# bifurcationkit/BifurcationKit.jl

Measured on NVIDIA H100. Metric: continuation steps/sec (SH2d PALC), higher is better.
Workload: dtype f64

## Files before the change

### bifurcationkit.jl_b200/csrc/bk_common.cuh

```cuda
#pragma once
#include <cuda_runtime.h>
#include <stdint.h>
#include <stdlib.h>
#include <string>
#include <unordered_map>
#include <vector>
#include "../../include/bk200.h"
#include <nvtx3/nvToolsExt.h>

struct BkRange {
  explicit BkRange(const char* name) { nvtxRangePushA(name); }
  ~BkRange() { nvtxRangePop(); }
};

#define BK_MAX_PAR 8
#define BK_NSM_FALLBACK 132

struct OpDesc {
  int kind;
  int nx, ny, nz;
  double cx, cy, cz;
  double par[BK_MAX_PAR];
  const double* u;
  double a0, a1;
// ... 34 lines not shown
  const double* sp;
  double a0, a1, l, nu;
  double spc;
};
#define PW_D 1

struct Precond {
  int kind = BK_PC_NONE;
  double a0 = 0, a1 = 0;
  double* lam[3] = {nullptr, nullptr, nullptr};
  int ttype[3] = {0, 0, 0};
  int fast[3] = {0, 0, 0};
  double2* ftw[3] = {nullptr, nullptr, nullptr};
  double2* fom[3] = {nullptr, nullptr, nullptr};
  double2* flam2[3] = {nullptr, nullptr, nullptr};
  bkg::Plan gplan[3] = {};
  double2* gwl[3] = {nullptr, nullptr, nullptr};
  double2* gph[3] = {nullptr, nullptr, nullptr};
  double* work = nullptr;
  double* work2 = nullptr;
  double* tri = nullptr;
  double2* tdft = nullptr;
  double po_r = 0, po_nu = 0, po_T = 0;
};

struct BkKindTraits {
  int ndims;
  int fields;
  int extra;
  bool jac_sym;
// ... 237 lines not shown
```

### bifurcationkit.jl_b200/csrc/bk_ctx.cu

```cuda
#include <cstdio>
#include <cstring>
#include <map>
#include <mutex>
#include <new>
#include "bk_common.cuh"

int bk_fail(bk_ctx* c, int code, const char* what, const char* file, int line) {
  if (c) {
    char buf[512];
    snprintf(buf, sizeof buf, "%s (%s:%d)", what, file, line);
    c->err = buf;
  }
  return code;
}

void bk_grant_smem(int device, const void* kern, size_t bytes) {
  static std::mutex mu;
  static std::map<std::pair<int, const void*>, size_t> granted;
  std::lock_guard<std::mutex> lk(mu);
  size_t& cur = granted[{device, kern}];
  if (bytes <= cur) return;
  cudaFuncSetAttribute(kern, cudaFuncAttributeMaxDynamicSharedMemorySize, (int)bytes);
  if (bytes > 48 * 1024) cudaFuncSetAttribute(kern, cudaFuncAttributePreferredSharedMemoryCarveout, 100);
  cur = bytes;
// ... 140 lines not shown
  }
  if (kind == BK_SH2D_PERIODIC) BK_TRY(bk_periodic_setup(c));
  BK_CUDA(c, cudaStreamSynchronize(c->stream));
  return BK_OK;
}

extern "C" int32_t bk_ctx_destroy(bk_ctx* c) {
  if (!c) return BK_OK;
  cudaSetDevice(c->device);
  if (c->stream) cudaStreamSynchronize(c->stream);
  double* bufs[] = {c->u_state, c->V, c->w, c->z, c->r, c->scales, c->gcoef, c->hcols, c->hcols2, c->partials,
                    c->red_out, c->phi, c->xpi, c->fcache, c->pc.work, c->pc.work2, c->pc.tri, c->Q, c->Q2, c->eig_dev};
  for (double* b : bufs)
    if (b) cudaFree(b);
  for (int d = 0; d < 3; ++d) {
    void* tabs[] = {c->pc.lam[d], c->pc.ftw[d], c->pc.fom[d], c->pc.flam2[d], c->pc.gwl[d], c->pc.gph[d]};
    for (void* t : tabs)
      if (t) cudaFree(t);
  }
  if (c->pc.tdft) cudaFree(c->pc.tdft);
  if (c->counters) cudaFree(c->counters);
  for (auto& kv : c->vec_live) cudaFree(kv.first);
  for (double* b : c->stage)
    if (b) cudaFree(b);
  for (double* b : c->tmp)
    if (b) cudaFree(b);
  if (c->h_pinned) cudaFreeHost(c->h_pinned);
  if (c->red_pinned) cudaFreeHost(c->red_pinned);
  if (c->coef_pinned) cudaFreeHost(c->coef_pinned);
  if (c->host_pinned) cudaFreeHost(c->host_pinned);
  if (c->eig_pinned) cudaFreeHost(c->eig_pinned);
// ... 253 lines not shown
```

### bifurcationkit.jl_b200/csrc/bk_fft_fast.cuh

```cuda
#pragma once
#include "bk_common.cuh"
#include "bk_async.cuh"

namespace bkf {

template <int LOGN_, int LOGE_>
struct Cfg {
  static constexpr int LOGN = LOGN_, LOGE = LOGE_;
  static constexpr int N = 1 << LOGN, E = 1 << LOGE, T = N / E;
  static constexpr int F = LOGN / LOGE, RB = LOGN % LOGE;
  static constexpr int NP = F + (RB ? 1 : 0);
  static constexpr int PP = (T >= 32) ? 2 : 64 / T;
  static constexpr int THREADS = T * PP;
  static constexpr int PB = LOGE == 5 ? (LOGN >= 10 ? 5 : 4) : LOGE == 4 ? 4 : LOGE == 3 ? ((LOGN == 9 || LOGN == 10) ? 3 : 0) : 0;
  __host__ __device__ static constexpr int pad(int i) { return i + (i >> 2) + (PB ? (i >> PB) : 0); }
  static constexpr int TPSM = LOGE == 5 ? 256 : LOGE == 4 ? 512 : LOGE == 3 ? 768 : 1024;
  static constexpr int MINB = TPSM / THREADS > 0 ? TPSM / THREADS : 1;
  static constexpr int MINB_P = MINB > 1 ? MINB - 1 : 1;
  static constexpr int NB = LOGE == 2 ? (LOGN <= 6 ? 0 : LOGN <= 8 ? 4 : LOGN <= 10 ? 6 : 8)
                          : LOGE == 3 ? (LOGN <= 6 ? 0 : LOGN <= 9 ? 3 : 6)
                          : LOGE == 4 ? (LOGN <= 8 ? 0 : 4)
                                      : (LOGN <= 10 ? 0 : 5);
  __host__ __device__ static constexpr int padn(int k) { return k + (k >> 2) + (NB ? (k >> NB) : 0); }
  static constexpr int SLOTS_POS = pad(N - 1) + 1, SLOTS_NAT = padn(N - 1) + 1;
  static constexpr int SLOTS = SLOTS_POS > SLOTS_NAT ? SLOTS_POS : SLOTS_NAT;
  static constexpr size_t SMEM_DATA = sizeof(double2) * (size_t)SLOTS * PP;
  __host__ __device__ static constexpr int logr(int p) { return p < F ? LOGE : RB; }
  __host__ __device__ static constexpr int logNp(int p) { return LOGN - LOGE * p; }
  __host__ __device__ static constexpr int logMp(int p) { return logNp(p) - logr(p); }
  __host__ __device__ static constexpr int tw_off(int p) {
    int o = 0;
    for (int q = 0; q < p; ++q) o += ((1 << logr(q)) - 1) << logMp(q);
    return o;
  }
  static constexpr int TW_TOTAL = tw_off(NP);
  static constexpr size_t SMEM = SMEM_DATA + sizeof(double2) * ((size_t)TW_TOTAL + N);
  static constexpr size_t SMEM_FUSED = SMEM + sizeof(double2) * (size_t)N;
  static_assert(LOGN >= LOGE + 1 && LOGN <= 11, "line length out of range");
  static_assert(THREADS <= 1024, "CTA too large");
};

template <class C>
__host__ __device__ inline int k_of_pos(int p) {
  int k = 0, sh = 0;
  for (int q = 0; q < C::NP; ++q) {
    const int d = (p >> C::logMp(q)) & ((1 << C::logr(q)) - 1);
    k |= d << sh;
    sh += C::logr(q);
  }
  return k;
}
template <class C>
// ... 80 lines not shown
    bfly_inv<H, S0, ESZ>(a);
    bfly_inv<H, S0 + H, ESZ>(a);
#pragma unroll
    for (int i = 0; i < H; ++i) {
      const double2 u = a[S0 + i], t = mul_w32<true>(a[S0 + i + H], i * (32 / R));
      a[S0 + i] = cadd(u, t);
      a[S0 + i + H] = csub(u, t);
    }
  }
}

struct Tables {
  const double2* tw;
  const double2* om;
  const double2* lam2;
};
template <class C, bool FUSED>
__device__ __forceinline__ Tables stage_tables(const Tables& g, double2* sm, unsigned long long* bar) {
  Tables t;
  double2* stw = sm + (size_t)C::SLOTS * C::PP;
  double2* som = stw + C::TW_TOTAL;
  double2* slam = som + C::N;
  if (threadIdx.x == 0) {
    mbar_init(bar, 1);
    fence_mbar_init();
    constexpr unsigned twb = 16u * C::TW_TOTAL, nb = 16u * C::N;
    mbar_arrive_expect_tx(bar, twb + nb + (FUSED ? nb : 0u));
    if (twb) bulk_g2s(stw, g.tw, twb, bar);
    bulk_g2s(som, g.om, nb, bar);
    if (FUSED) bulk_g2s(slam, g.lam2, nb, bar);
  }
  t.tw = stw;
  t.om = som;
  t.lam2 = slam;
  return t;
}

struct Geom {
  long long es;
  long long os;
  int nb;
  int nouter;
};

struct Symbol {
  const double* lam_b;
  const double* lam_o;
  double shift;
  double scale;
// ... 128 lines not shown
    for (int i = 0; i < C::E; ++i) a[i] = make_double2(v0 ? __ldg(base + (long long)row_of<C>(i, tau) * es) : 0.0, 0.0);
  }
}
template <class C>
__device__ __forceinline__ void strided_store(const double2 (&a)[C::E], double* __restrict__ base, long long es, int tau, bool v0,
                                              bool v1) {
  if (v1) {
#pragma unroll
    for (int i = 0; i < C::E; ++i) *reinterpret_cast<double2*>(base + (long long)row_of<C>(i, tau) * es) = a[i];
  } else if (v0) {
#pragma unroll
    for (int i = 0; i < C::E; ++i) base[(long long)row_of<C>(i, tau) * es] = a[i].x;
  }
}

#define BKF_BOUNDS(C, PERIODIC) __launch_bounds__(C::THREADS, (PERIODIC) ? C::MINB_P : C::MINB)

__device__ __forceinline__ double rcp_nr(double x) {
  double r;
  asm("rcp.approx.ftz.f64 %0, %1;" : "=d"(r) : "d"(x));
  double e = fma(-x, r, 1.0);
  r = fma(r, e, r);
  e = fma(-x, r, 1.0);
  return fma(r, e, r);
}
__device__ __forceinline__ double per_symbol(const Symbol& sy, double lam) {
  const double t = 1.0 + lam, l1 = t * t;
  return sy.neg ? -sy.scale * l1 : sy.scale * rcp_nr(l1 + sy.shift);
}

template <class C, int MODE>
static __global__ void BKF_BOUNDS(C, MODE == 3) k_strided(const double* __restrict__ in, double* __restrict__ out, Geom g, Tables tbg, Symbol sy) {
  extern __shared__ __align__(128) double2 sm_fast[];
  __shared__ __align__(8) unsigned long long tbar;
  double2* sm = sm_fast;
  const Tables tb = stage_tables<C, MODE == 2 || MODE == 3>(tbg, sm, &tbar);
  const int tid = threadIdx.x, pr = tid % C::PP, tau = tid / C::PP;
  __syncthreads();
  bk_pdl_sync();
  const int col = (blockIdx.x * C::PP + pr) * 2, o = blockIdx.y;
  const bool v0 = col < g.nb, v1 = col + 1 < g.nb;
  const long long off = (long long)o * g.os + col;
  if ((MODE == 2 || MODE == 3) && sy.tail_n > 0 && blockIdx.x == 0 && blockIdx.y == 0 && tid < sy.tail_n)
    sy.tail_dst[tid] = sy.tail_src[tid];
  double2 a[C::E];
  if (MODE == 3) {
#pragma unroll
    for (int i = 0; i < C::E; ++i) {
      const double* p = in + off + (long long)(i * C::T + tau) * g.es;
      a[i] = v1 ? __ldg(reinterpret_cast<const double2*>(p)) : make_double2(v0 ? __ldg(p) : 0.0, 0.0);
    }
    mbar_wait(&tbar, 0);
    fwd_passes<C, 0>(a, sm, tb, tau, pr);
    const bool nyq = blockIdx.x == 0 && pr == 0;
    if (blockIdx.x == 0) {
      park<C>(a, sm, tau, pr);
      __syncthreads();
      if (nyq) {
        const double l0 = __ldg(sy.lam_b), ln = __ldg(sy.lam_b + (g.nb >> 1));
#pragma unroll
        for (int reg = 0; reg < C::E; ++reg) {
          int k;
          const double2 z = a[reg], zp = partner<C>(sm, reg_pos<C>(tau, reg), pr, k);
          const double ly = tb.lam2[reg * C::T + tau].x;
          const double s0 = per_symbol(sy, l0 + ly), sn = per_symbol(sy, ln + ly);
          const double hp = 0.5 * (s0 + sn), hm = 0.5 * (s0 - sn);
          a[reg] = make_double2(fma(hp, z.x, hm * zp.x), fma(hp, z.y, -(hm * zp.y)));
        }
      }
      __syncthreads();
    }
    if (!nyq) {
      const double lq = v0 ? __ldg(sy.lam_b + (col >> 1)) : 0.0;
#pragma unroll
      for (int reg = 0; reg < C::E; ++reg) {
        const double s = per_symbol(sy, lq + tb.lam2[reg * C::T + tau].x);
        a[reg] = make_double2(s * a[reg].x, s * a[reg].y);
      }
    }
    inv_passes<C, C::NP - 1>(a, sm, tb, tau, pr);
#pragma unroll
    for (int i = 0; i < C::E; ++i) {
      double* p = out + off + (long long)(i * C::T + tau) * g.es;
      if (v1) *reinterpret_cast<double2*>(p) = a[i];
      else if (v0) *p = a[i].x;
    }
    return;
  }
  if (MODE != 1) {
    strided_load<C>(a, in + off, g.es, tau, v0, v1);
    mbar_wait(&tbar, 0);
    fwd_passes<C, 0>(a, sm, tb, tau, pr);
    park<C>(a, sm, tau, pr);
    __syncthreads();
  }
  if (MODE == 0) {
#pragma unroll
    for (int reg = 0; reg < C::E; ++reg) {
      int k;
      const double2 z = a[reg], zp = partner<C>(sm, reg_pos<C>(tau, reg), pr, k);
      const double2 w = tb.om[reg * C::T + tau];
      const double sx = z.x + zp.x, sy_ = z.y - zp.y;
      const double dx = z.x - zp.x, dy = z.y + zp.y;
      const double c1 = fma(w.x, sx, -(w.y * sy_)), c2 = fma(w.x, dy, w.y * dx);
      double* p = out + off + (long long)k * g.es;
      if (v1) *reinterpret_cast<double2*>(p) = make_double2(c1, c2);
      else if (v0) *p = c1;
    }
    return;
  }
  if (MODE == 1) {
#pragma unroll
    for (int reg = 0; reg < C::E; ++reg) {
      const int k = k_of_pos<C>(reg_pos<C>(tau, reg));
      const double* p = in + off + (long long)k * g.es;
      a[reg] = v1 ? __ldg(reinterpret_cast<const double2*>(p)) : make_double2(v0 ? __ldg(p) : 0.0, 0.0);
    }
    mbar_wait(&tbar, 0);
    park<C>(a, sm, tau, pr);
    __syncthreads();
#pragma unroll
    for (int reg = 0; reg < C::E; ++reg) {
      int k;
      double2 dn = partner<C>(sm, reg_pos<C>(tau, reg), pr, k);
      if (k == 0) dn = make_double2(0.0, 0.0);
      const double2 w = tb.om[reg * C::T + tau];
      a[reg] = cmulc(make_double2(a[reg].x + dn.y, a[reg].y - dn.x), w);
    }
    __syncthreads();
  }
  if (MODE == 2) {
    const double lo = sy.lam_o ? __ldg(sy.lam_o + o) : 0.0;
    const double cA = 1.0 + lo + (v0 ? __ldg(sy.lam_b + col) : 0.0), cB = 1.0 + lo + (v1 ? __ldg(sy.lam_b + col + 1) : 0.0);
#pragma unroll
    for (int reg = 0; reg < C::E; ++reg) {
      int k;
      const double2 z = a[reg], zp = partner<C>(sm, reg_pos<C>(tau, reg), pr, k);
      const double2 w = tb.om[reg * C::T + tau];
      const double2 l2 = tb.lam2[reg * C::T + tau];
      const double2 A1 = cmul(make_double2(z.x + zp.x, z.y - zp.y), w);
      const double2 A2 = cmul(make_double2(z.y + zp.y, zp.x - z.x), w);
      double t = cA + l2.x;
      const double s1k = fma(t, t, sy.shift);
      t = cA + l2.y;
      const double s1n = fma(t, t, sy.shift);
      t = cB + l2.x;
      const double s2k = fma(t, t, sy.shift);
      t = cB + l2.y;
      const double s2n = fma(t, t, sy.shift);
      const double r1 = sy.scale * __drcp_rn(s1k * s1n), r2 = sy.scale * __drcp_rn(s2k * s2n);
      const double h1x = A1.x * (r1 * s1n), h1y = A1.y * (r1 * s1k);
      const double h2x = A2.x * (r2 * s2n), h2y = A2.y * (r2 * s2k);
      a[reg] = cmulc(make_double2(h1x - h2y, h1y + h2x), w);
    }
    __syncthreads();
  }
  inv_passes<C, C::NP - 1>(a, sm, tb, tau, pr);
  strided_store<C>(a, out + off, g.es, tau, v0, v1);
}

template <class C>
__device__ __forceinline__ int nslot(int k, int pr) { return C::padn(k) * C::PP + pr; }

__device__ __forceinline__ double pw_c(const PerPw& pw, double u) { return fma(u, fma(-3.0, u, 2.0 * pw.nu), pw.l); }
__device__ __forceinline__ double pw_d(const PerPw& pw, double u) { return fma(pw.a1, pw.spc + pw_c(pw, u), pw.a0); }
__device__ __forceinline__ double pw_out(const PerPw& pw, double y, const double* v, const double* u, int m, double s) {
  switch (pw.epi) {
    case PW_RESID: {
      const double x = __ldg(v + m);
      return fma(x, fma(x, pw.nu - x, pw.l), y);
    }
    case PW_JVP: return fma(fma(pw.a1, pw_c(pw, __ldg(u + m)), pw.a0), s * __ldg(v + m), y);
    case PW_FLEFT: return fma(-pw.a1 * s, __ldg(v + m), y);
    case PW_FRIGHT: return fma(pw_d(pw, __ldg(u + m)), y, -pw.a1 * s * __ldg(v + m));
    default: return y;
  }
}

template <class C, int MODE>
static __global__ void BKF_BOUNDS(C, MODE == 2) k_contig(const double* __restrict__ in, double* __restrict__ out, Geom g, Tables tbg, PerPw pw) {
  extern __shared__ __align__(128) double2 sm_fast[];
  __shared__ __align__(8) unsigned long long tbar;
  double2* sm = sm_fast;
  const Tables tb = stage_tables<C, false>(tbg, sm, &tbar);
  const int tid = threadIdx.x, pr = tid % C::PP, tau = tid / C::PP;
  __syncthreads();
  bk_pdl_sync();
  const long long lineA = ((long long)blockIdx.x * C::PP + pr) * 2, lineB = lineA + 1;
  const bool vA = lineA < g.nb, vB = lineB < g.nb;
  const double* inA = in + lineA * g.os;
  const double* inB = in + lineB * g.os;
  double* outA = out + lineA * g.os;
  double* outB = out + lineB * g.os;
  double2 a[C::E];
  if (MODE == 2) {
    const double s = pw.sp ? __ldg(pw.sp) : 1.0;
#pragma unroll
    for (int i = 0; i < C::E; ++i) {
      const int m = i * C::T + tau;
      double xa = vA ? __ldg(inA + m) : 0.0, xb = vB ? __ldg(inB + m) : 0.0;
      if (pw.pro == PW_D) {
        xa *= vA ? pw_d(pw, __ldg(pw.u + lineA * g.os + m)) : 0.0;
        xb *= vB ? pw_d(pw, __ldg(pw.u + lineB * g.os + m)) : 0.0;
      }
      a[i] = make_double2(s * xa, s * xb);
    }
    mbar_wait(&tbar, 0);
    fwd_passes<C, 0>(a, sm, tb, tau, pr);
    park<C>(a, sm, tau, pr);
    __syncthreads();
    double2 b[C::E];
#pragma unroll
    for (int reg = 0; reg < C::E; ++reg) {
      int k;
      const double2 z = a[reg], zp = partner<C>(sm, reg_pos<C>(tau, reg), pr, k);
      a[reg] = make_double2(0.5 * (z.x + zp.x), 0.5 * (z.y + zp.y));
      b[reg] = make_double2(0.5 * (z.y - zp.y), 0.5 * (zp.x - z.x));
    }
    __syncthreads();
#pragma unroll
    for (int reg = 0; reg < C::E; ++reg) {
      const int k = k_of_pos<C>(reg_pos<C>(tau, reg));
      if (k == 0) sm[nslot<C>(0, pr)] = a[reg];
      else if (k == C::N / 2) sm[nslot<C>(1, pr)] = a[reg];
      else if (k < C::N / 2) {
        sm[nslot<C>(2 * k, pr)] = a[reg];
        sm[nslot<C>(2 * k + 1, pr)] = b[reg];
      }
    }
    __syncthreads();
#pragma unroll
    for (int i = 0; i < C::E; ++i) {
      const int p = i * C::T + tau;
      const double2 d = sm[nslot<C>(p, pr)];
      if (vA) outA[p] = d.x;
      if (vB) outB[p] = d.y;
    }
    return;
  }
  if (MODE == 3) {
#pragma unroll
    for (int i = 0; i < C::E; ++i) {
      const int p = i * C::T + tau;
      sm[nslot<C>(p, pr)] = make_double2(vA ? __ldg(inA + p) : 0.0, vB ? __ldg(inB + p) : 0.0);
    }
    mbar_wait(&tbar, 0);
    __syncthreads();
#pragma unroll
    for (int reg = 0; reg < C::E; ++reg) {
      const int k = k_of_pos<C>(reg_pos<C>(tau, reg)), kk = k <= C::N / 2 ? k : C::N - k;
      double2 xa, xb;
      if (kk == 0 || kk == C::N / 2) {
        const double2 d = sm[nslot<C>(kk ? 1 : 0, pr)];
        xa = make_double2(d.x, 0.0);
        xb = make_double2(d.y, 0.0);
      } else {
        const double2 re = sm[nslot<C>(2 * kk, pr)], im = sm[nslot<C>(2 * kk + 1, pr)];
        xa = make_double2(re.x, k == kk ? im.x : -im.x);
        xb = make_double2(re.y, k == kk ? im.y : -im.y);
      }
      a[reg] = make_double2(xa.x - xb.y, xa.y + xb.x);
    }
    __syncthreads();
    inv_passes<C, C::NP - 1>(a, sm, tb, tau, pr);
    const double s = pw.sp ? __ldg(pw.sp) : 1.0;
    const double* vrA = pw.v + lineA * g.os;
    const double* vrB = pw.v + lineB * g.os;
    const double* urA = pw.u ? pw.u + lineA * g.os : nullptr;
    const double* urB = pw.u ? pw.u + lineB * g.os : nullptr;
#pragma unroll
    for (int i = 0; i < C::E; ++i) {
      const int m = i * C::T + tau;
      if (vA) outA[m] = pw_out(pw, a[i].x, vrA, urA, m, s);
      if (vB) outB[m] = pw_out(pw, a[i].y, vrB, urB, m, s);
    }
    return;
  }
  if (MODE == 0) {
#pragma unroll
    for (int i = 0; i < C::E; ++i) {
      const int e = row_of<C>(i, tau);
      a[i] = make_double2(vA ? __ldg(inA + e) : 0.0, vB ? __ldg(inB + e) : 0.0);
    }
    mbar_wait(&tbar, 0);
    fwd_passes<C, 0>(a, sm, tb, tau, pr);
    park<C>(a, sm, tau, pr);
    __syncthreads();
#pragma unroll
    for (int reg = 0; reg < C::E; ++reg) {
      int k;
      const double2 z = a[reg], zp = partner<C>(sm, reg_pos<C>(tau, reg), pr, k);
      const double2 w = tb.om[reg * C::T + tau];
      const double sx = z.x + zp.x, sy_ = z.y - zp.y, dx = z.x - zp.x, dy = z.y + zp.y;
      a[reg] = make_double2(fma(w.x, sx, -(w.y * sy_)), fma(w.x, dy, w.y * dx));
    }
    __syncthreads();
#pragma unroll
    for (int reg = 0; reg < C::E; ++reg) sm[nslot<C>(k_of_pos<C>(reg_pos<C>(tau, reg)), pr)] = a[reg];
    __syncthreads();
#pragma unroll
    for (int i = 0; i < C::E; ++i) {
      const int k = i * C::T + tau;
      const double2 d = sm[nslot<C>(k, pr)];
      if (vA) outA[k] = d.x;
      if (vB) outB[k] = d.y;
    }
  } else {
#pragma unroll
    for (int i = 0; i < C::E; ++i) {
      const int k = i * C::T + tau;
      sm[nslot<C>(k, pr)] = make_double2(vA ? __ldg(inA + k) : 0.0, vB ? __ldg(inB + k) : 0.0);
    }
    mbar_wait(&tbar, 0);
    __syncthreads();
#pragma unroll
    for (int reg = 0; reg < C::E; ++reg) {
      const int k = k_of_pos<C>(reg_pos<C>(tau, reg)), nk = (C::N - k) & (C::N - 1);
      const double2 w = tb.om[reg * C::T + tau];
      const double2 d = sm[nslot<C>(k, pr)];
      double2 dn = sm[nslot<C>(nk, pr)];
      if (k == 0) dn = make_double2(0.0, 0.0);
      a[reg] = cmulc(make_double2(d.x + dn.y, d.y - dn.x), w);
    }
    __syncthreads();
    inv_passes<C, C::NP - 1>(a, sm, tb, tau, pr);
#pragma unroll
    for (int i = 0; i < C::E; ++i) {
      const int e = row_of<C>(i, tau);
      if (vA) outA[e] = a[i].x;
      if (vB) outB[e] = a[i].y;
    }
  }
}
#endif

template <class C>
static inline void build_tables(std::vector<double>& tw, std::vector<double>& om, std::vector<double>& lam2, const double* lam) {
  const long double PI = 3.14159265358979323846264338327950288L;
  tw.assign(2 * (size_t)C::TW_TOTAL, 0.0);
  for (int p = 0; p < C::NP - 1; ++p) {
    const int r = 1 << C::logr(p), M = 1 << C::logMp(p), Np = 1 << C::logNp(p);
    for (int q = 1; q < r; ++q)
      for (int b = 0; b < M; ++b) {
        const long double ang = -2.0L * PI * (long double)((long long)b * q % Np) / Np;
        const size_t i = (size_t)C::tw_off(p) + (size_t)(q - 1) * M + b;
        tw[2 * i] = (double)cosl(ang);
        tw[2 * i + 1] = (double)sinl(ang);
      }
  }
  om.assign(2 * (size_t)C::N, 0.0);
  lam2.assign(2 * (size_t)C::N, 0.0);
  const int LR = C::logr(C::NP - 1), R = 1 << LR;
  for (int reg = 0; reg < C::E; ++reg)
    for (int tau = 0; tau < C::T; ++tau) {
      const int u = reg >> LR, j = reg & (R - 1);
      const int pos = ((tau + C::T * u) << LR) + brev_c(j, LR);
      const int k = k_of_pos<C>(pos), nk = (C::N - k) & (C::N - 1);
      const size_t i = (size_t)reg * C::T + tau;
      om[2 * i] = (double)cosl(-PI * k / (2.0L * C::N));
      om[2 * i + 1] = (double)sinl(-PI * k / (2.0L * C::N));
      if (lam) {
        lam2[2 * i] = lam[k];
        lam2[2 * i + 1] = lam[nk];
      }
    }
}
// ... 2 lines not shown
```

### bifurcationkit.jl_b200/csrc/bk_precond.cu

```cuda
#include <cmath>
#include <cstdlib>
#include <utility>
#include <vector>
#include "bk_common.cuh"

#include "bk_fft_fast.cuh"
#include "bk_fft_gen.cuh"

static __global__ void __launch_bounds__(256) k_sh_symbol_div(double* __restrict__ a, int nx, int ny, int nz,
                                                              const double* __restrict__ lx, const double* __restrict__ ly,
                                                              const double* __restrict__ lz, double shift, double scale) {
  const long long total = (long long)nx * ny * nz;
  for (long long q = (long long)blockIdx.x * blockDim.x + threadIdx.x; q < total; q += (long long)gridDim.x * blockDim.x) {
    int i = (int)(q % nx), j = (int)((q / nx) % ny), k = (int)(q / ((long long)nx * ny));
    double t = 1.0 + lx[i] + ly[j] + (lz ? lz[k] : 0.0);
    a[q] = a[q] * scale / (t * t + shift);
  }
}
static __global__ void __launch_bounds__(256) k_helmholtz_symbol_div(double* __restrict__ a, int nx, int ny, long long nblocks,
                                                                     const double* __restrict__ lx,
                                                                     const double* __restrict__ ly, double a0, double a1) {
  const long long n = (long long)nx * ny, total = n * nblocks;
  for (long long q = (long long)blockIdx.x * blockDim.x + threadIdx.x; q < total; q += (long long)gridDim.x * blockDim.x) {
    long long g = q % n;
// ... 108 lines not shown
    case 8: { using FC = bkf::Cfg<8, LE>; __VA_ARGS__; } break;                        \
    case 9: { using FC = bkf::Cfg<9, LE>; __VA_ARGS__; } break;                        \
    case 10: { using FC = bkf::Cfg<10, LE>; __VA_ARGS__; } break;                      \
    default: { using FC = bkf::Cfg<11, LE>; __VA_ARGS__; } break;                      \
  }
#define BKF_DISPATCH(LOGN, ...)                                                        \
  switch (fast_loge(1LL << (LOGN))) {                                                               \
    case 2: BKF_DISPATCH_N(2, LOGN, __VA_ARGS__) break;                                \
    case 3: BKF_DISPATCH_N(3, LOGN, __VA_ARGS__) break;                                \
    case 4: BKF_DISPATCH_N(4, LOGN, __VA_ARGS__) break;                                \
    default: BKF_DISPATCH_N(5, LOGN, __VA_ARGS__) break;                               \
  }

template <class FC>
static int fast_setup(bk_ctx* c, int d, const double* lam_host) {
  std::vector<double> tw, om, lam2;
  bkf::build_tables<FC>(tw, om, lam2, lam_host);
  Precond& pc = c->pc;
  if (tw.empty()) tw.assign(2, 0.0);
  BK_TRY(upload(c, (void**)&pc.ftw[d], tw.data(), 8 * tw.size()));
  BK_TRY(upload(c, (void**)&pc.fom[d], om.data(), 8 * om.size()));
  BK_TRY(upload(c, (void**)&pc.flam2[d], lam2.data(), 8 * lam2.size()));
  return BK_OK;
}

template <class FC>
static int fast_launch(bk_ctx* c, int d, bool strided, int mode, const double* in, double* out, const bkf::Geom& g,
                       const bkf::Symbol* sy, const PerPw* pw = nullptr) {
  Precond& pc = c->pc;
  bkf::Tables tb{pc.ftw[d], pc.fom[d], pc.flam2[d]};
  bkf::Symbol s0{};
  if (sy) s0 = *sy;
  PerPw p0{};
  if (pw) p0 = *pw;
  if (strided) {
    static decltype(&bkf::k_strided<FC, 0>) const kern[4] = {bkf::k_strided<FC, 0>, bkf::k_strided<FC, 1>, bkf::k_strided<FC, 2>,
                                                             bkf::k_strided<FC, 3>};
    const dim3 grid((g.nb + 2 * FC::PP - 1) / (2 * FC::PP), g.nouter);
    return bk_launch(c, kern[mode], grid, dim3(FC::THREADS), mode >= 2 ? FC::SMEM_FUSED : FC::SMEM, in, out, g, tb, s0);
  }
  static decltype(&bkf::k_contig<FC, 0>) const kern[4] = {bkf::k_contig<FC, 0>, bkf::k_contig<FC, 1>, bkf::k_contig<FC, 2>,
                                                          bkf::k_contig<FC, 3>};
  const dim3 grid((unsigned)((g.nb + 2 * FC::PP - 1) / (2 * FC::PP)));
  return bk_launch(c, kern[mode], grid, dim3(FC::THREADS), FC::SMEM, in, out, g, tb, p0);
}

static void factorize(int L, bkg::Plan& pl) {
  pl.npass = 0;
  while (L % 4 == 0 && pl.npass < BKG_MAXPASS) {
    pl.radix[pl.npass++] = 4;
    L /= 4;
  }
  for (int p = 2; L > 1 && pl.npass < BKG_MAXPASS; ++p)
    while (L % p == 0 && pl.npass < BKG_MAXPASS) {
      pl.radix[pl.npass++] = p;
      L /= p;
    }
}
// ... 333 lines not shown
```

Baseline: 4.057.

## Make fast FFT kernels persistent with occupancy-sized grids and smem-aware launch bounds

Converts the strided and contiguous fast FFT kernels into grid-stride persistent loops over line groups. The grid is capped at SMs times measured resident blocks, so the twiddle tables staged once in shared memory are reused across groups. Launch bounds now derive min blocks from shared-memory footprint and a register-pressure heuristic rather than a fixed threads-per-SM ratio. Contiguous mode 0 now does a natural-order post-twiddle with a new omn table. This adds per-group syncthreads and changes register limits, which may cause spills or fewer resident blocks.

```diff
diff --git a/bifurcationkit.jl_b200/csrc/bk_common.cuh b/bifurcationkit.jl_b200/csrc/bk_common.cuh
--- a/bifurcationkit.jl_b200/csrc/bk_common.cuh
+++ b/bifurcationkit.jl_b200/csrc/bk_common.cuh
@@ -72,6 +72,7 @@
   double2* ftw[3] = {nullptr, nullptr, nullptr};
   double2* fom[3] = {nullptr, nullptr, nullptr};
   double2* flam2[3] = {nullptr, nullptr, nullptr};
+  double2* fomn[3] = {nullptr, nullptr, nullptr};
   bkg::Plan gplan[3] = {};
   double2* gwl[3] = {nullptr, nullptr, nullptr};
   double2* gph[3] = {nullptr, nullptr, nullptr};
diff --git a/bifurcationkit.jl_b200/csrc/bk_ctx.cu b/bifurcationkit.jl_b200/csrc/bk_ctx.cu
--- a/bifurcationkit.jl_b200/csrc/bk_ctx.cu
+++ b/bifurcationkit.jl_b200/csrc/bk_ctx.cu
@@ -178,7 +178,7 @@
   for (double* b : bufs)
     if (b) cudaFree(b);
   for (int d = 0; d < 3; ++d) {
-    void* tabs[] = {c->pc.lam[d], c->pc.ftw[d], c->pc.fom[d], c->pc.flam2[d], c->pc.gwl[d], c->pc.gph[d]};
+    void* tabs[] = {c->pc.lam[d], c->pc.ftw[d], c->pc.fom[d], c->pc.flam2[d], c->pc.fomn[d], c->pc.gwl[d], c->pc.gph[d]};
     for (void* t : tabs)
       if (t) cudaFree(t);
   }
diff --git a/bifurcationkit.jl_b200/csrc/bk_fft_fast.cuh b/bifurcationkit.jl_b200/csrc/bk_fft_fast.cuh
--- a/bifurcationkit.jl_b200/csrc/bk_fft_fast.cuh
+++ b/bifurcationkit.jl_b200/csrc/bk_fft_fast.cuh
@@ -15,8 +15,6 @@
   static constexpr int PB = LOGE == 5 ? (LOGN >= 10 ? 5 : 4) : LOGE == 4 ? 4 : LOGE == 3 ? ((LOGN == 9 || LOGN == 10) ? 3 : 0) : 0;
   __host__ __device__ static constexpr int pad(int i) { return i + (i >> 2) + (PB ? (i >> PB) : 0); }
   static constexpr int TPSM = LOGE == 5 ? 256 : LOGE == 4 ? 512 : LOGE == 3 ? 768 : 1024;
-  static constexpr int MINB = TPSM / THREADS > 0 ? TPSM / THREADS : 1;
-  static constexpr int MINB_P = MINB > 1 ? MINB - 1 : 1;
   static constexpr int NB = LOGE == 2 ? (LOGN <= 6 ? 0 : LOGN <= 8 ? 4 : LOGN <= 10 ? 6 : 8)
                           : LOGE == 3 ? (LOGN <= 6 ? 0 : LOGN <= 9 ? 3 : 6)
                           : LOGE == 4 ? (LOGN <= 8 ? 0 : 4)
@@ -36,6 +34,13 @@
   static constexpr int TW_TOTAL = tw_off(NP);
   static constexpr size_t SMEM = SMEM_DATA + sizeof(double2) * ((size_t)TW_TOTAL + N);
   static constexpr size_t SMEM_FUSED = SMEM + sizeof(double2) * (size_t)N;
+  static constexpr int SMEM_SM = 228 * 1024, SMEM_CTA_RESERVED = 1024;
+  __host__ __device__ static constexpr int minb(size_t smem, int heavy) {
+    const int by_smem = (int)(SMEM_SM / (smem + SMEM_CTA_RESERVED));
+    const int by_regs = (heavy == 0 ? TPSM : heavy == 1 || LOGE != 2 ? TPSM * 3 / 4 : TPSM * 5 / 8) / THREADS;
+    const int m = by_smem < by_regs ? by_smem : by_regs;
+    return m > 1 ? (m < 32 ? m : 32) : 1;
+  }
   static_assert(LOGN >= LOGE + 1 && LOGN <= 11, "line length out of range");
   static_assert(THREADS <= 1024, "CTA too large");
 };
@@ -146,8 +151,9 @@
   const double2* tw;
   const double2* om;
   const double2* lam2;
+  const double2* omn;
 };
-template <class C, bool FUSED>
+template <class C, bool FUSED, bool NAT = false>
 __device__ __forceinline__ Tables stage_tables(const Tables& g, double2* sm, unsigned long long* bar) {
   Tables t;
   double2* stw = sm + (size_t)C::SLOTS * C::PP;
@@ -159,12 +165,13 @@
     constexpr unsigned twb = 16u * C::TW_TOTAL, nb = 16u * C::N;
     mbar_arrive_expect_tx(bar, twb + nb + (FUSED ? nb : 0u));
     if (twb) bulk_g2s(stw, g.tw, twb, bar);
-    bulk_g2s(som, g.om, nb, bar);
+    bulk_g2s(som, NAT ? g.omn : g.om, nb, bar);
     if (FUSED) bulk_g2s(slam, g.lam2, nb, bar);
   }
   t.tw = stw;
   t.om = som;
   t.lam2 = slam;
+  t.omn = som;
   return t;
 }
 
@@ -323,7 +330,13 @@
   }
 }
 
-#define BKF_BOUNDS(C, PERIODIC) __launch_bounds__(C::THREADS, (PERIODIC) ? C::MINB_P : C::MINB)
+__device__ __forceinline__ int tid_opaque() {
+  int t;
+  asm volatile("mov.u32 %0, %%tid.x;" : "=r"(t));
+  return t;
+}
+
+#define BKF_BOUNDS(C, SMEM, HEAVY) __launch_bounds__(C::THREADS, C::minb(SMEM, HEAVY))
 
 __device__ __forceinline__ double rcp_nr(double x) {
   double r;
@@ -339,133 +352,138 @@
 }
 
 template <class C, int MODE>
-static __global__ void BKF_BOUNDS(C, MODE == 3) k_strided(const double* __restrict__ in, double* __restrict__ out, Geom g, Tables tbg, Symbol sy) {
+static __global__ void BKF_BOUNDS(C, MODE >= 2 ? C::SMEM_FUSED : C::SMEM, MODE == 2 ? 2 : MODE != 0) k_strided(const double* __restrict__ in, double* __restrict__ out, Geom g, Tables tbg, Symbol sy) {
   extern __shared__ __align__(128) double2 sm_fast[];
   __shared__ __align__(8) unsigned long long tbar;
   double2* sm = sm_fast;
   const Tables tb = stage_tables<C, MODE == 2 || MODE == 3>(tbg, sm, &tbar);
-  const int tid = threadIdx.x, pr = tid % C::PP, tau = tid / C::PP;
   __syncthreads();
   bk_pdl_sync();
-  const int col = (blockIdx.x * C::PP + pr) * 2, o = blockIdx.y;
-  const bool v0 = col < g.nb, v1 = col + 1 < g.nb;
-  const long long off = (long long)o * g.os + col;
-  if ((MODE == 2 || MODE == 3) && sy.tail_n > 0 && blockIdx.x == 0 && blockIdx.y == 0 && tid < sy.tail_n)
-    sy.tail_dst[tid] = sy.tail_src[tid];
-  double2 a[C::E];
-  if (MODE == 3) {
-#pragma unroll
-    for (int i = 0; i < C::E; ++i) {
-      const double* p = in + off + (long long)(i * C::T + tau) * g.es;
-      a[i] = v1 ? __ldg(reinterpret_cast<const double2*>(p)) : make_double2(v0 ? __ldg(p) : 0.0, 0.0);
-    }
-    mbar_wait(&tbar, 0);
-    fwd_passes<C, 0>(a, sm, tb, tau, pr);
-    const bool nyq = blockIdx.x == 0 && pr == 0;
-    if (blockIdx.x == 0) {
+  const int xb = (g.nb + 2 * C::PP - 1) / (2 * C::PP), ng = xb * g.nouter;
+  for (int grp = blockIdx.x; grp < ng; grp += gridDim.x) {
+    __syncthreads();
+    const int tid = tid_opaque(), pr = tid % C::PP, tau = tid / C::PP;
+    const int bx = grp % xb, o = grp / xb;
+    const int col = (bx * C::PP + pr) * 2;
+    const bool v0 = col < g.nb, v1 = col + 1 < g.nb;
+    const long long off = (long long)o * g.os + col;
+    if ((MODE == 2 || MODE == 3) && sy.tail_n > 0 && bx == 0 && o == 0 && tid < sy.tail_n)
+      sy.tail_dst[tid] = sy.tail_src[tid];
+    double2 a[C::E];
+    if (MODE == 3) {
+#pragma unroll
+      for (int i = 0; i < C::E; ++i) {
+        const double* p = in + off + (long long)(i * C::T + tau) * g.es;
+        a[i] = v1 ? __ldg(reinterpret_cast<const double2*>(p)) : make_double2(v0 ? __ldg(p) : 0.0, 0.0);
+      }
+      mbar_wait(&tbar, 0);
+      fwd_passes<C, 0>(a, sm, tb, tau, pr);
+      const bool nyq = bx == 0 && pr == 0;
+      if (bx == 0) {
+        park<C>(a, sm, tau, pr);
+        __syncthreads();
+        if (nyq) {
+          const double l0 = __ldg(sy.lam_b), ln = __ldg(sy.lam_b + (g.nb >> 1));
+#pragma unroll
+          for (int reg = 0; reg < C::E; ++reg) {
+            int k;
+            const double2 z = a[reg], zp = partner<C>(sm, reg_pos<C>(tau, reg), pr, k);
+            const double ly = tb.lam2[reg * C::T + tau].x;
+            const double s0 = per_symbol(sy, l0 + ly), sn = per_symbol(sy, ln + ly);
+            const double hp = 0.5 * (s0 + sn), hm = 0.5 * (s0 - sn);
+            a[reg] = make_double2(fma(hp, z.x, hm * zp.x), fma(hp, z.y, -(hm * zp.y)));
+          }
+        }
+        __syncthreads();
+      }
+      if (!nyq) {
+        const double lq = v0 ? __ldg(sy.lam_b + (col >> 1)) : 0.0;
+#pragma unroll
+        for (int reg = 0; reg < C::E; ++reg) {
+          const double s = per_symbol(sy, lq + tb.lam2[reg * C::T + tau].x);
+          a[reg] = make_double2(s * a[reg].x, s * a[reg].y);
+        }
+      }
+      inv_passes<C, C::NP - 1>(a, sm, tb, tau, pr);
+#pragma unroll
+      for (int i = 0; i < C::E; ++i) {
+        double* p = out + off + (long long)(i * C::T + tau) * g.es;
+        if (v1) *reinterpret_cast<double2*>(p) = a[i];
+        else if (v0) *p = a[i].x;
+      }
+      continue;
+    }
+    if (MODE != 1) {
+      strided_load<C>(a, in + off, g.es, tau, v0, v1);
+      mbar_wait(&tbar, 0);
+      fwd_passes<C, 0>(a, sm, tb, tau, pr);
       park<C>(a, sm, tau, pr);
       __syncthreads();
-      if (nyq) {
-        const double l0 = __ldg(sy.lam_b), ln = __ldg(sy.lam_b + (g.nb >> 1));
-#pragma unroll
-        for (int reg = 0; reg < C::E; ++reg) {
-          int k;
-          const double2 z = a[reg], zp = partner<C>(sm, reg_pos<C>(tau, reg), pr, k);
-          const double ly = tb.lam2[reg * C::T + tau].x;
-          const double s0 = per_symbol(sy, l0 + ly), sn = per_symbol(sy, ln + ly);
-          const double hp = 0.5 * (s0 + sn), hm = 0.5 * (s0 - sn);
-          a[reg] = make_double2(fma(hp, z.x, hm * zp.x), fma(hp, z.y, -(hm * zp.y)));
-        }
-      }
-      __syncthreads();
-    }
-    if (!nyq) {
-      const double lq = v0 ? __ldg(sy.lam_b + (col >> 1)) : 0.0;
-#pragma unroll
-      for (int reg = 0; reg < C::E; ++reg) {
-        const double s = per_symbol(sy, lq + tb.lam2[reg * C::T + tau].x);
-        a[reg] = make_double2(s * a[reg].x, s * a[reg].y);
-      }
+    }
+    if (MODE == 0) {
+#pragma unroll
+      for (int reg = 0; reg < C::E; ++reg) {
+        int k;
+        const double2 z = a[reg], zp = partner<C>(sm, reg_pos<C>(tau, reg), pr, k);
+        const double2 w = tb.om[reg * C::T + tau];
+        const double sx = z.x + zp.x, sy_ = z.y - zp.y;
+        const double dx = z.x - zp.x, dy = z.y + zp.y;
+        const double c1 = fma(w.x, sx, -(w.y * sy_)), c2 = fma(w.x, dy, w.y * dx);
+        double* p = out + off + (long long)k * g.es;
+        if (v1) *reinterpret_cast<double2*>(p) = make_double2(c1, c2);
+        else if (v0) *p = c1;
+      }
+      continue;
+    }
+    if (MODE == 1) {
+#pragma unroll
+      for (int reg = 0; reg < C::E; ++reg) {
+        const int k = k_of_pos<C>(reg_pos<C>(tau, reg));
+        const double* p = in + off + (long long)k * g.es;
+        a[reg] = v1 ? __ldg(reinterpret_cast<const double2*>(p)) : make_double2(v0 ? __ldg(p) : 0.0, 0.0);
+      }
+      mbar_wait(&tbar, 0);
+      park<C>(a, sm, tau, pr);
+      __syncthreads();
+#pragma unroll
+      for (int reg = 0; reg < C::E; ++reg) {
+        int k;
+        double2 dn = partner<C>(sm, reg_pos<C>(tau, reg), pr, k);
+        if (k == 0) dn = make_double2(0.0, 0.0);
+        const double2 w = tb.om[reg * C::T + tau];
+        a[reg] = cmulc(make_double2(a[reg].x + dn.y, a[reg].y - dn.x), w);
+      }
+      __syncthreads();
+    }
+    if (MODE == 2) {
+      const double lo = sy.lam_o ? __ldg(sy.lam_o + o) : 0.0;
+      const double cA = 1.0 + lo + (v0 ? __ldg(sy.lam_b + col) : 0.0), cB = 1.0 + lo + (v1 ? __ldg(sy.lam_b + col + 1) : 0.0);
+#pragma unroll
+      for (int reg = 0; reg < C::E; ++reg) {
+        int k;
+        const double2 z = a[reg], zp = partner<C>(sm, reg_pos<C>(tau, reg), pr, k);
+        const double2 w = tb.om[reg * C::T + tau];
+        const double2 l2 = tb.lam2[reg * C::T + tau];
+        const double2 A1 = cmul(make_double2(z.x + zp.x, z.y - zp.y), w);
+        const double2 A2 = cmul(make_double2(z.y + zp.y, zp.x - z.x), w);
+        double t = cA + l2.x;
+        const double s1k = fma(t, t, sy.shift);
+        t = cA + l2.y;
+        const double s1n = fma(t, t, sy.shift);
+        t = cB + l2.x;
+        const double s2k = fma(t, t, sy.shift);
+        t = cB + l2.y;
+        const double s2n = fma(t, t, sy.shift);
+        const double r1 = sy.scale * __drcp_rn(s1k * s1n), r2 = sy.scale * __drcp_rn(s2k * s2n);
+        const double h1x = A1.x * (r1 * s1n), h1y = A1.y * (r1 * s1k);
+        const double h2x = A2.x * (r2 * s2n), h2y = A2.y * (r2 * s2k);
+        a[reg] = cmulc(make_double2(h1x - h2y, h1y + h2x), w);
+      }
+      __syncthreads();
     }
     inv_passes<C, C::NP - 1>(a, sm, tb, tau, pr);
-#pragma unroll
-    for (int i = 0; i < C::E; ++i) {
-      double* p = out + off + (long long)(i * C::T + tau) * g.es;
-      if (v1) *reinterpret_cast<double2*>(p) = a[i];
-      else if (v0) *p = a[i].x;
-    }
-    return;
-  }
-  if (MODE != 1) {
-    strided_load<C>(a, in + off, g.es, tau, v0, v1);
-    mbar_wait(&tbar, 0);
-    fwd_passes<C, 0>(a, sm, tb, tau, pr);
-    park<C>(a, sm, tau, pr);
-    __syncthreads();
-  }
-  if (MODE == 0) {
-#pragma unroll
-    for (int reg = 0; reg < C::E; ++reg) {
-      int k;
-      const double2 z = a[reg], zp = partner<C>(sm, reg_pos<C>(tau, reg), pr, k);
-      const double2 w = tb.om[reg * C::T + tau];
-      const double sx = z.x + zp.x, sy_ = z.y - zp.y;
-      const double dx = z.x - zp.x, dy = z.y + zp.y;
-      const double c1 = fma(w.x, sx, -(w.y * sy_)), c2 = fma(w.x, dy, w.y * dx);
-      double* p = out + off + (long long)k * g.es;
-      if (v1) *reinterpret_cast<double2*>(p) = make_double2(c1, c2);
-      else if (v0) *p = c1;
-    }
-    return;
-  }
-  if (MODE == 1) {
-#pragma unroll
-    for (int reg = 0; reg < C::E; ++reg) {
-      const int k = k_of_pos<C>(reg_pos<C>(tau, reg));
-      const double* p = in + off + (long long)k * g.es;
-      a[reg] = v1 ? __ldg(reinterpret_cast<const double2*>(p)) : make_double2(v0 ? __ldg(p) : 0.0, 0.0);
-    }
-    mbar_wait(&tbar, 0);
-    park<C>(a, sm, tau, pr);
-    __syncthreads();
-#pragma unroll
-    for (int reg = 0; reg < C::E; ++reg) {
-      int k;
-      double2 dn = partner<C>(sm, reg_pos<C>(tau, reg), pr, k);
-      if (k == 0) dn = make_double2(0.0, 0.0);
-      const double2 w = tb.om[reg * C::T + tau];
-      a[reg] = cmulc(make_double2(a[reg].x + dn.y, a[reg].y - dn.x), w);
-    }
-    __syncthreads();
-  }
-  if (MODE == 2) {
-    const double lo = sy.lam_o ? __ldg(sy.lam_o + o) : 0.0;
-    const double cA = 1.0 + lo + (v0 ? __ldg(sy.lam_b + col) : 0.0), cB = 1.0 + lo + (v1 ? __ldg(sy.lam_b + col + 1) : 0.0);
-#pragma unroll
-    for (int reg = 0; reg < C::E; ++reg) {
-      int k;
-      const double2 z = a[reg], zp = partner<C>(sm, reg_pos<C>(tau, reg), pr, k);
-      const double2 w = tb.om[reg * C::T + tau];
-      const double2 l2 = tb.lam2[reg * C::T + tau];
-      const double2 A1 = cmul(make_double2(z.x + zp.x, z.y - zp.y), w);
-      const double2 A2 = cmul(make_double2(z.y + zp.y, zp.x - z.x), w);
-      double t = cA + l2.x;
-      const double s1k = fma(t, t, sy.shift);
-      t = cA + l2.y;
-      const double s1n = fma(t, t, sy.shift);
-      t = cB + l2.x;
-      const double s2k = fma(t, t, sy.shift);
-      t = cB + l2.y;
-      const double s2n = fma(t, t, sy.shift);
-      const double r1 = sy.scale * __drcp_rn(s1k * s1n), r2 = sy.scale * __drcp_rn(s2k * s2n);
-      const double h1x = A1.x * (r1 * s1n), h1y = A1.y * (r1 * s1k);
-      const double h2x = A2.x * (r2 * s2n), h2y = A2.y * (r2 * s2k);
-      a[reg] = cmulc(make_double2(h1x - h2y, h1y + h2x), w);
-    }
-    __syncthreads();
-  }
-  inv_passes<C, C::NP - 1>(a, sm, tb, tau, pr);
-  strided_store<C>(a, out + off, g.es, tau, v0, v1);
+    strided_store<C>(a, out + off, g.es, tau, v0, v1);
+  }
 }
 
 template <class C>
@@ -487,164 +505,162 @@
 }
 
 template <class C, int MODE>
-static __global__ void BKF_BOUNDS(C, MODE == 2) k_contig(const double* __restrict__ in, double* __restrict__ out, Geom g, Tables tbg, PerPw pw) {
+static __global__ void BKF_BOUNDS(C, C::SMEM, MODE == 2 ? 1 : 0) k_contig(const double* __restrict__ in, double* __restrict__ out, Geom g, Tables tbg, PerPw pw) {
   extern __shared__ __align__(128) double2 sm_fast[];
   __shared__ __align__(8) unsigned long long tbar;
   double2* sm = sm_fast;
-  const Tables tb = stage_tables<C, false>(tbg, sm, &tbar);
-  const int tid = threadIdx.x, pr = tid % C::PP, tau = tid / C::PP;
+  const Tables tb = stage_tables<C, false, MODE == 0>(tbg, sm, &tbar);
   __syncthreads();
   bk_pdl_sync();
-  const long long lineA = ((long long)blockIdx.x * C::PP + pr) * 2, lineB = lineA + 1;
-  const bool vA = lineA < g.nb, vB = lineB < g.nb;
-  const double* inA = in + lineA * g.os;
-  const double* inB = in + lineB * g.os;
-  double* outA = out + lineA * g.os;
-  double* outB = out + lineB * g.os;
-  double2 a[C::E];
-  if (MODE == 2) {
-    const double s = pw.sp ? __ldg(pw.sp) : 1.0;
-#pragma unroll
-    for (int i = 0; i < C::E; ++i) {
-      const int m = i * C::T + tau;
-      double xa = vA ? __ldg(inA + m) : 0.0, xb = vB ? __ldg(inB + m) : 0.0;
-      if (pw.pro == PW_D) {
-        xa *= vA ? pw_d(pw, __ldg(pw.u + lineA * g.os + m)) : 0.0;
-        xb *= vB ? pw_d(pw, __ldg(pw.u + lineB * g.os + m)) : 0.0;
-      }
-      a[i] = make_double2(s * xa, s * xb);
-    }
-    mbar_wait(&tbar, 0);
-    fwd_passes<C, 0>(a, sm, tb, tau, pr);
-    park<C>(a, sm, tau, pr);
+  const int ng = (g.nb + 2 * C::PP - 1) / (2 * C::PP);
+  for (int grp = blockIdx.x; grp < ng; grp += gridDim.x) {
     __syncthreads();
-    double2 b[C::E];
-#pragma unroll
-    for (int reg = 0; reg < C::E; ++reg) {
-      int k;
-      const double2 z = a[reg], zp = partner<C>(sm, reg_pos<C>(tau, reg), pr, k);
-      a[reg] = make_double2(0.5 * (z.x + zp.x), 0.5 * (z.y + zp.y));
-      b[reg] = make_double2(0.5 * (z.y - zp.y), 0.5 * (zp.x - z.x));
-    }
-    __syncthreads();
-#pragma unroll
-    for (int reg = 0; reg < C::E; ++reg) {
-      const int k = k_of_pos<C>(reg_pos<C>(tau, reg));
-      if (k == 0) sm[nslot<C>(0, pr)] = a[reg];
-      else if (k == C::N / 2) sm[nslot<C>(1, pr)] = a[reg];
-      else if (k < C::N / 2) {
-        sm[nslot<C>(2 * k, pr)] = a[reg];
-        sm[nslot<C>(2 * k + 1, pr)] = b[reg];
-      }
-    }
-    __syncthreads();
-#pragma unroll
-    for (int i = 0; i < C::E; ++i) {
-      const int p = i * C::T + tau;
-      const double2 d = sm[nslot<C>(p, pr)];
-      if (vA) outA[p] = d.x;
-      if (vB) outB[p] = d.y;
-    }
-    return;
-  }
-  if (MODE == 3) {
-#pragma unroll
-    for (int i = 0; i < C::E; ++i) {
-      const int p = i * C::T + tau;
-      sm[nslot<C>(p, pr)] = make_double2(vA ? __ldg(inA + p) : 0.0, vB ? __ldg(inB + p) : 0.0);
-    }
-    mbar_wait(&tbar, 0);
-    __syncthreads();
-#pragma unroll
-    for (int reg = 0; reg < C::E; ++reg) {
-      const int k = k_of_pos<C>(reg_pos<C>(tau, reg)), kk = k <= C::N / 2 ? k : C::N - k;
-      double2 xa, xb;
-      if (kk == 0 || kk == C::N / 2) {
-        const double2 d = sm[nslot<C>(kk ? 1 : 0, pr)];
-        xa = make_double2(d.x, 0.0);
-        xb = make_double2(d.y, 0.0);
-      } else {
-        const double2 re = sm[nslot<C>(2 * kk, pr)], im = sm[nslot<C>(2 * kk + 1, pr)];
-        xa = make_double2(re.x, k == kk ? im.x : -im.x);
-        xb = make_double2(re.y, k == kk ? im.y : -im.y);
-      }
-      a[reg] = make_double2(xa.x - xb.y, xa.y + xb.x);
-    }
-    __syncthreads();
-    inv_passes<C, C::NP - 1>(a, sm, tb, tau, pr);
-    const double s = pw.sp ? __ldg(pw.sp) : 1.0;
-    const double* vrA = pw.v + lineA * g.os;
-    const double* vrB = pw.v + lineB * g.os;
-    const double* urA = pw.u ? pw.u + lineA * g.os : nullptr;
-    const double* urB = pw.u ? pw.u + lineB * g.os : nullptr;
-#pragma unroll
-    for (int i = 0; i < C::E; ++i) {
-      const int m = i * C::T + tau;
-      if (vA) outA[m] = pw_out(pw, a[i].x, vrA, urA, m, s);
-      if (vB) outB[m] = pw_out(pw, a[i].y, vrB, urB, m, s);
-    }
-    return;
-  }
-  if (MODE == 0) {
-#pragma unroll
-    for (int i = 0; i < C::E; ++i) {
-      const int e = row_of<C>(i, tau);
-      a[i] = make_double2(vA ? __ldg(inA + e) : 0.0, vB ? __ldg(inB + e) : 0.0);
-    }
-    mbar_wait(&tbar, 0);
-    fwd_passes<C, 0>(a, sm, tb, tau, pr);
-    park<C>(a, sm, tau, pr);
-    __syncthreads();
-#pragma unroll
-    for (int reg = 0; reg < C::E; ++reg) {
-      int k;
-      const double2 z = a[reg], zp = partner<C>(sm, reg_pos<C>(tau, reg), pr, k);
-      const double2 w = tb.om[reg * C::T + tau];
-      const double sx = z.x + zp.x, sy_ = z.y - zp.y, dx = z.x - zp.x, dy = z.y + zp.y;
-      a[reg] = make_double2(fma(w.x, sx, -(w.y * sy_)), fma(w.x, dy, w.y * dx));
-    }
-    __syncthreads();
-#pragma unroll
-    for (int reg = 0; reg < C::E; ++reg) sm[nslot<C>(k_of_pos<C>(reg_pos<C>(tau, reg)), pr)] = a[reg];
-    __syncthreads();
-#pragma unroll
-    for (int i = 0; i < C::E; ++i) {
-      const int k = i * C::T + tau;
-      const double2 d = sm[nslot<C>(k, pr)];
-      if (vA) outA[k] = d.x;
-      if (vB) outB[k] = d.y;
-    }
-  } else {
-#pragma unroll
-    for (int i = 0; i < C::E; ++i) {
-      const int k = i * C::T + tau;
-      sm[nslot<C>(k, pr)] = make_double2(vA ? __ldg(inA + k) : 0.0, vB ? __ldg(inB + k) : 0.0);
-    }
-    mbar_wait(&tbar, 0);
-    __syncthreads();
-#pragma unroll
-    for (int reg = 0; reg < C::E; ++reg) {
-      const int k = k_of_pos<C>(reg_pos<C>(tau, reg)), nk = (C::N - k) & (C::N - 1);
-      const double2 w = tb.om[reg * C::T + tau];
-      const double2 d = sm[nslot<C>(k, pr)];
-      double2 dn = sm[nslot<C>(nk, pr)];
-      if (k == 0) dn = make_double2(0.0, 0.0);
-      a[reg] = cmulc(make_double2(d.x + dn.y, d.y - dn.x), w);
-    }
-    __syncthreads();
-    inv_passes<C, C::NP - 1>(a, sm, tb, tau, pr);
-#pragma unroll
-    for (int i = 0; i < C::E; ++i) {
-      const int e = row_of<C>(i, tau);
-      if (vA) outA[e] = a[i].x;
-      if (vB) outB[e] = a[i].y;
+    const int tid = tid_opaque(), pr = tid % C::PP, tau = tid / C::PP;
+    const long long lineA = ((long long)grp * C::PP + pr) * 2, lineB = lineA + 1;
+    const bool vA = lineA < g.nb, vB = lineB < g.nb;
+    const double* inA = in + lineA * g.os;
+    const double* inB = in + lineB * g.os;
+    double* outA = out + lineA * g.os;
+    double* outB = out + lineB * g.os;
+    double2 a[C::E];
+    if (MODE == 2) {
+      const double s = pw.sp ? __ldg(pw.sp) : 1.0;
+#pragma unroll
+      for (int i = 0; i < C::E; ++i) {
+        const int m = i * C::T + tau;
+        double xa = vA ? __ldg(inA + m) : 0.0, xb = vB ? __ldg(inB + m) : 0.0;
+        if (pw.pro == PW_D) {
+          xa *= vA ? pw_d(pw, __ldg(pw.u + lineA * g.os + m)) : 0.0;
+          xb *= vB ? pw_d(pw, __ldg(pw.u + lineB * g.os + m)) : 0.0;
+        }
+        a[i] = make_double2(s * xa, s * xb);
+      }
+      mbar_wait(&tbar, 0);
+      fwd_passes<C, 0>(a, sm, tb, tau, pr);
+      park<C>(a, sm, tau, pr);
+      __syncthreads();
+      double2 b[C::E];
+#pragma unroll
+      for (int reg = 0; reg < C::E; ++reg) {
+        int k;
+        const double2 z = a[reg], zp = partner<C>(sm, reg_pos<C>(tau, reg), pr, k);
+        a[reg] = make_double2(0.5 * (z.x + zp.x), 0.5 * (z.y + zp.y));
+        b[reg] = make_double2(0.5 * (z.y - zp.y), 0.5 * (zp.x - z.x));
+      }
+      __syncthreads();
+#pragma unroll
+      for (int reg = 0; reg < C::E; ++reg) {
+        const int k = k_of_pos<C>(reg_pos<C>(tau, reg));
+        if (k == 0) sm[nslot<C>(0, pr)] = a[reg];
+        else if (k == C::N / 2) sm[nslot<C>(1, pr)] = a[reg];
+        else if (k < C::N / 2) {
+          sm[nslot<C>(2 * k, pr)] = a[reg];
+          sm[nslot<C>(2 * k + 1, pr)] = b[reg];
+        }
+      }
+      __syncthreads();
+#pragma unroll
+      for (int i = 0; i < C::E; ++i) {
+        const int p = i * C::T + tau;
+        const double2 d = sm[nslot<C>(p, pr)];
+        if (vA) outA[p] = d.x;
+        if (vB) outB[p] = d.y;
+      }
+      continue;
+    }
+    if (MODE == 3) {
+#pragma unroll
+      for (int i = 0; i < C::E; ++i) {
+        const int p = i * C::T + tau;
+        sm[nslot<C>(p, pr)] = make_double2(vA ? __ldg(inA + p) : 0.0, vB ? __ldg(inB + p) : 0.0);
+      }
+      mbar_wait(&tbar, 0);
+      __syncthreads();
+#pragma unroll
+      for (int reg = 0; reg < C::E; ++reg) {
+        const int k = k_of_pos<C>(reg_pos<C>(tau, reg)), kk = k <= C::N / 2 ? k : C::N - k;
+        double2 xa, xb;
+        if (kk == 0 || kk == C::N / 2) {
+          const double2 d = sm[nslot<C>(kk ? 1 : 0, pr)];
+          xa = make_double2(d.x, 0.0);
+          xb = make_double2(d.y, 0.0);
+        } else {
+          const double2 re = sm[nslot<C>(2 * kk, pr)], im = sm[nslot<C>(2 * kk + 1, pr)];
+          xa = make_double2(re.x, k == kk ? im.x : -im.x);
+          xb = make_double2(re.y, k == kk ? im.y : -im.y);
+        }
+        a[reg] = make_double2(xa.x - xb.y, xa.y + xb.x);
+      }
+      __syncthreads();
+      inv_passes<C, C::NP - 1>(a, sm, tb, tau, pr);
+      const double s = pw.sp ? __ldg(pw.sp) : 1.0;
+      const double* vrA = pw.v + lineA * g.os;
+      const double* vrB = pw.v + lineB * g.os;
+      const double* urA = pw.u ? pw.u + lineA * g.os : nullptr;
+      const double* urB = pw.u ? pw.u + lineB * g.os : nullptr;
+#pragma unroll
+      for (int i = 0; i < C::E; ++i) {
+        const int m = i * C::T + tau;
+        if (vA) outA[m] = pw_out(pw, a[i].x, vrA, urA, m, s);
+        if (vB) outB[m] = pw_out(pw, a[i].y, vrB, urB, m, s);
+      }
+      continue;
+    }
+    if (MODE == 0) {
+#pragma unroll
+      for (int i = 0; i < C::E; ++i) {
+        const int e = row_of<C>(i, tau);
+        a[i] = make_double2(vA ? __ldg(inA + e) : 0.0, vB ? __ldg(inB + e) : 0.0);
+      }
+      mbar_wait(&tbar, 0);
+      fwd_passes<C, 0>(a, sm, tb, tau, pr);
+      __syncthreads();
+#pragma unroll
+      for (int reg = 0; reg < C::E; ++reg) sm[nslot<C>(k_of_pos<C>(reg_pos<C>(tau, reg)), pr)] = a[reg];
+      __syncthreads();
+#pragma unroll
+      for (int i = 0; i < C::E; ++i) {
+        const int k = i * C::T + tau;
+        const double2 z = sm[nslot<C>(k, pr)], zp = sm[nslot<C>((C::N - k) & (C::N - 1), pr)];
+        const double2 w = tb.omn[k];
+        const double sx = z.x + zp.x, sy_ = z.y - zp.y, dx = z.x - zp.x, dy = z.y + zp.y;
+        const double c1 = fma(w.x, sx, -(w.y * sy_)), c2 = fma(w.x, dy, w.y * dx);
+        if (vA) outA[k] = c1;
+        if (vB) outB[k] = c2;
+      }
+    } else {
+#pragma unroll
+      for (int i = 0; i < C::E; ++i) {
+        const int k = i * C::T + tau;
+        sm[nslot<C>(k, pr)] = make_double2(vA ? __ldg(inA + k) : 0.0, vB ? __ldg(inB + k) : 0.0);
+      }
+      mbar_wait(&tbar, 0);
+      __syncthreads();
+#pragma unroll
+      for (int reg = 0; reg < C::E; ++reg) {
+        const int k = k_of_pos<C>(reg_pos<C>(tau, reg)), nk = (C::N - k) & (C::N - 1);
+        const double2 w = tb.om[reg * C::T + tau];
+        const double2 d = sm[nslot<C>(k, pr)];
+        double2 dn = sm[nslot<C>(nk, pr)];
+        if (k == 0) dn = make_double2(0.0, 0.0);
+        a[reg] = cmulc(make_double2(d.x + dn.y, d.y - dn.x), w);
+      }
+      __syncthreads();
+      inv_passes<C, C::NP - 1>(a, sm, tb, tau, pr);
+#pragma unroll
+      for (int i = 0; i < C::E; ++i) {
+        const int e = row_of<C>(i, tau);
+        if (vA) outA[e] = a[i].x;
+        if (vB) outB[e] = a[i].y;
+      }
     }
   }
 }
 #endif
 
 template <class C>
-static inline void build_tables(std::vector<double>& tw, std::vector<double>& om, std::vector<double>& lam2, const double* lam) {
+static inline void build_tables(std::vector<double>& tw, std::vector<double>& om, std::vector<double>& lam2, std::vector<double>& omn,
+                                const double* lam) {
   const long double PI = 3.14159265358979323846264338327950288L;
   tw.assign(2 * (size_t)C::TW_TOTAL, 0.0);
   for (int p = 0; p < C::NP - 1; ++p) {
@@ -659,6 +675,11 @@
   }
   om.assign(2 * (size_t)C::N, 0.0);
   lam2.assign(2 * (size_t)C::N, 0.0);
+  omn.assign(2 * (size_t)C::N, 0.0);
+  for (int k = 0; k < C::N; ++k) {
+    omn[2 * (size_t)k] = (double)cosl(-PI * k / (2.0L * C::N));
+    omn[2 * (size_t)k + 1] = (double)sinl(-PI * k / (2.0L * C::N));
+  }
   const int LR = C::logr(C::NP - 1), R = 1 << LR;
   for (int reg = 0; reg < C::E; ++reg)
     for (int tau = 0; tau < C::T; ++tau) {
diff --git a/bifurcationkit.jl_b200/csrc/bk_precond.cu b/bifurcationkit.jl_b200/csrc/bk_precond.cu
--- a/bifurcationkit.jl_b200/csrc/bk_precond.cu
+++ b/bifurcationkit.jl_b200/csrc/bk_precond.cu
@@ -146,34 +146,50 @@
 
 template <class FC>
 static int fast_setup(bk_ctx* c, int d, const double* lam_host) {
-  std::vector<double> tw, om, lam2;
-  bkf::build_tables<FC>(tw, om, lam2, lam_host);
+  std::vector<double> tw, om, lam2, omn;
+  bkf::build_tables<FC>(tw, om, lam2, omn, lam_host);
   Precond& pc = c->pc;
   if (tw.empty()) tw.assign(2, 0.0);
   BK_TRY(upload(c, (void**)&pc.ftw[d], tw.data(), 8 * tw.size()));
   BK_TRY(upload(c, (void**)&pc.fom[d], om.data(), 8 * om.size()));
   BK_TRY(upload(c, (void**)&pc.flam2[d], lam2.data(), 8 * lam2.size()));
-  return BK_OK;
+  BK_TRY(upload(c, (void**)&pc.fomn[d], omn.data(), 8 * omn.size()));
+  return BK_OK;
+}
+
+template <class FC, class K>
+static unsigned fast_grid(bk_ctx* c, K kern, int slot, size_t smem, long long groups) {
+  static int per_sm[8] = {0};
+  bk_ensure_smem(c, kern, smem);
+  if (!per_sm[slot]) {
+    int nb = 0;
+    if (cudaOccupancyMaxActiveBlocksPerMultiprocessor(&nb, kern, FC::THREADS, smem) != cudaSuccess || nb < 1) nb = 1;
+    per_sm[slot] = nb;
+  }
+  const long long resident = (long long)c->nsm * per_sm[slot];
+  return (unsigned)(groups < resident ? groups : resident);
 }
 
 template <class FC>
 static int fast_launch(bk_ctx* c, int d, bool strided, int mode, const double* in, double* out, const bkf::Geom& g,
                        const bkf::Symbol* sy, const PerPw* pw = nullptr) {
   Precond& pc = c->pc;
-  bkf::Tables tb{pc.ftw[d], pc.fom[d], pc.flam2[d]};
+  bkf::Tables tb{pc.ftw[d], pc.fom[d], pc.flam2[d], pc.fomn[d]};
   bkf::Symbol s0{};
   if (sy) s0 = *sy;
   PerPw p0{};
   if (pw) p0 = *pw;
+  const long long groups = (g.nb + 2 * FC::PP - 1) / (2 * FC::PP) * (strided ? (long long)g.nouter : 1LL);
   if (strided) {
     static decltype(&bkf::k_strided<FC, 0>) const kern[4] = {bkf::k_strided<FC, 0>, bkf::k_strided<FC, 1>, bkf::k_strided<FC, 2>,
                                                              bkf::k_strided<FC, 3>};
-    const dim3 grid((g.nb + 2 * FC::PP - 1) / (2 * FC::PP), g.nouter);
-    return bk_launch(c, kern[mode], grid, dim3(FC::THREADS), mode >= 2 ? FC::SMEM_FUSED : FC::SMEM, in, out, g, tb, s0);
+    const size_t smem = mode >= 2 ? FC::SMEM_FUSED : FC::SMEM;
+    const dim3 grid(fast_grid<FC>(c, kern[mode], 4 + mode, smem, groups));
+    return bk_launch(c, kern[mode], grid, dim3(FC::THREADS), smem, in, out, g, tb, s0);
   }
   static decltype(&bkf::k_contig<FC, 0>) const kern[4] = {bkf::k_contig<FC, 0>, bkf::k_contig<FC, 1>, bkf::k_contig<FC, 2>,
                                                           bkf::k_contig<FC, 3>};
-  const dim3 grid((unsigned)((g.nb + 2 * FC::PP - 1) / (2 * FC::PP)));
+  const dim3 grid(fast_grid<FC>(c, kern[mode], mode, FC::SMEM, groups));
   return bk_launch(c, kern[mode], grid, dim3(FC::THREADS), FC::SMEM, in, out, g, tb, p0);
 }
 
```

Result: no change. 4.087, median of 6 (+0.7%).
